# ThomasHelfer/multimodal-supernovae

Hardware: AMD Instinct MI355X
Metric: contrastive pairs/sec (image+light-curve) at global batch 1024, 1/2/4/8 GPUs (higher is better)
Workload: dtype f32; 1 GPU; ViT-S/8 image tower (64x64x3, build-defined) + reference light-curve transformer (T=200, emb 64, 8 heads, depth 5, 2 bands) -> enc_dim 128, symmetric InfoNCE with all-gathered global negatives, RAdam; full train step; per_gpu_batch=1024, global_batch=1024, parallelism=dp1, launch=eager, gemm_precision=bf16x6

## Files before the change

include/msn_hip.h:

```cpp
#ifndef MSN_HIP_H
#define MSN_HIP_H

#include <stddef.h>
#include <stdint.h>

#ifdef __cplusplus
extern "C" {
#endif

#define MSN_OK 0
#define MSN_ERR_SHAPE 1
#define MSN_ERR_HIP 2

typedef void* msn_stream_t;

int msn_version(void);
const char* msn_last_error(void);
int msn_clock_probe(unsigned long long* out2, int microseconds, msn_stream_t stream);
int msn_device_count(void);

#define MSN_OP_N 0
#define MSN_OP_T 1
#define MSN_EPI_NONE 0
#define MSN_EPI_RELU 1
// ... 86 lines not shown
                       msn_stream_t stream);
size_t msn_time_embed_bwd_workspace_bytes(int64_t B, int e, int nband);
int msn_time_embed_bwd(const float* dy, const float* x, int64_t B, int T, int e, int nband, float* dw,
                       float* dbw, float* dband, void* ws, size_t ws_bytes, msn_stream_t stream);

#define MSN_POOL_MEAN 0
#define MSN_POOL_MAX 1
int msn_masked_pool_fwd(const float* x, const uint8_t* mask, int64_t B, int T, int e, int mode, float* out,
                        int* argmax, float* count, msn_stream_t stream);
int msn_masked_pool_bwd(const float* dout, const uint8_t* mask, int64_t B, int T, int e, int mode,
                        const int* argmax, const float* count, float* dx, msn_stream_t stream);
int msn_mask_tokens(const float* x, const uint8_t* mask, int64_t rows, int e, float* y, msn_stream_t stream);

int msn_add_rows(float* dst, int64_t ldd, const float* src, int64_t lds, int64_t rows, int cols, msn_stream_t stream);

size_t msn_plane_bytes(int64_t R, int64_t C, int planes);
size_t msn_plane_split_colsum_workspace_bytes(int64_t R, int64_t C);
int msn_plane_split(const float* x, int64_t ldx, int64_t R, int64_t C, int planes, int transposed, void* out, float* colsum,
                    void* ws, size_t ws_bytes, msn_stream_t stream);
typedef struct msn_split_item {
    const float* x;
    int64_t ldx, R, C;
    int transposed;
    void* out;
} msn_split_item;
int msn_plane_split_list(int n, const msn_split_item* items, int planes, msn_stream_t stream);
int msn_plane_merge(const void* planes_in, int planes, int64_t R, int64_t C, float* y, int64_t ldy, msn_stream_t stream);
size_t msn_pgemm_nt_colsum_workspace_bytes(int64_t M, int N);
size_t msn_pgemm_nt_workspace_bytes(int64_t M, int N, int K, int planes, int c_planes, int epilogue, int want_colsum);
int msn_set_pgemm_tail_split(int enabled);
int msn_pgemm_nt(int64_t M, int N, int K, int planes, const void* A, const void* B, void* C, int64_t ldc, int c_planes,
                 const float* bias, int epilogue, float* aux, int64_t ldaux, float* colsum_out, void* ws, size_t ws_bytes,
                 msn_stream_t stream);
size_t msn_pgemm_tn_workspace_bytes(int64_t M, int N, int K, int planes);
int msn_pgemm_tn(int64_t M, int N, int K, int planes, const void* A, const void* B, float* C, int64_t ldc, void* ws,
                 size_t ws_bytes, msn_stream_t stream);
int msn_layernorm_fwd_planes(const float* x, int64_t ldx, int64_t rows, int cols, const float* gamma, const float* beta,
                             float eps, int planes, void* y_planes, float* y, int64_t ldy, float* mean, float* rstd,
                             msn_stream_t stream);
int msn_layernorm_bwd_planes(const float* dy, int64_t lddy, const float* x, int64_t ldx, int64_t rows, int cols,
                             const float* mean, const float* rstd, const float* gamma, const float* add, int64_t ldadd,
                             float* dx, int64_t lddx, int planes, void* dx_planes, float* dgamma, float* dbeta,
                             float* dx_colsum, void* ws, size_t ws_bytes, msn_stream_t stream);
int msn_attention_fwd_planes(const float* qkv, int64_t ldqkv, const uint8_t* key_mask, int B, int H, int T, int head_dim,
                             float scale, float* out, int64_t ldo, float* lse, int planes, void* out_planes, msn_stream_t stream);
size_t msn_attention_bwd_planes_workspace_bytes(int B, int H, int head_dim);
int msn_attention_bwd_planes(const float* qkv, int64_t ldqkv, const uint8_t* key_mask, int B, int H, int T, int head_dim,
                             float scale, const float* out, int64_t ldo, const float* lse, const float* dout, int64_t ldd,
                             int planes, void* dqkv_planes, float* colsum_out, void* ws, size_t ws_bytes,
                             msn_stream_t stream);
int msn_plane_split_f16(const float* x, int64_t ldx, int64_t R, int64_t C, int transposed, void* out, float* scale,
                        int reuse_scale, float* colsum, void* ws, size_t ws_bytes, msn_stream_t stream);
int msn_pgemm_nt_f16(int64_t M, int N, int K, const void* A, const float* scaleA, const void* B, const float* scaleB, float* C,
                     int64_t ldc, const float* bias, int epilogue, float* aux, int64_t ldaux, float* colsum_out, void* ws,
                     size_t ws_bytes, msn_stream_t stream);
int msn_pgemm_tn_f16(int64_t M, int N, int K, const void* A, const float* scaleA, const void* B, const float* scaleB, float* C,
                     int64_t ldc, void* ws, size_t ws_bytes, msn_stream_t stream);

int msn_ffn_supported(int64_t M, int emb, int hidden);
int msn_ffn_fwd(const float* x, int64_t ldx, int64_t M, int emb, int hidden, const void* w1_planes, const void* w2t_planes,
                const float* c1, const float* c2, float* z, int64_t ldz, msn_stream_t stream);
size_t msn_ffn_bwd_workspace_bytes(int64_t M, int emb, int hidden);
int msn_ffn_bwd(const float* x, int64_t ldx, const float* dz, int64_t lddz, int64_t M, int emb, int hidden, const void* w1_planes,
                const void* w2t_planes, const float* c1, float* dx, int64_t lddx, float* dw1, float* dc1, float* dw2, float* dc2,
                void* ws, size_t ws_bytes, msn_stream_t stream);

// ... 224 lines not shown
```

multimodal_supernovae_amd/_lib.py:

```python
import ctypes
import os

import torch

_HERE = os.path.dirname(os.path.abspath(__file__))
LIB_PATH = os.environ.get("MSN_HIP_LIB") or os.path.join(_HERE, "lib", "libmsn_hip.so")

c_i64 = ctypes.c_int64
c_int = ctypes.c_int
c_f32 = ctypes.c_float
c_f64 = ctypes.c_double
c_ptr = ctypes.c_void_p
c_size = ctypes.c_size_t

SIGNATURES = {
    "msn_version": (c_int, []),
    "msn_last_error": (ctypes.c_char_p, []),
    "msn_clock_probe": (c_int, [c_ptr, c_int, c_ptr]),
    "msn_ffn_supported": (c_int, [c_i64, c_int, c_int]),
    "msn_ffn_fwd": (c_int, [c_ptr, c_i64, c_i64, c_int, c_int, c_ptr, c_ptr, c_ptr, c_ptr, c_ptr, c_i64, c_ptr]),
    "msn_ffn_bwd_workspace_bytes": (c_size, [c_i64, c_int, c_int]),
    "msn_ffn_bwd": (c_int, [c_ptr, c_i64, c_ptr, c_i64, c_i64, c_int, c_int, c_ptr, c_ptr, c_ptr, c_ptr, c_i64, c_ptr, c_ptr, c_ptr,
                            c_ptr, c_ptr, c_size, c_ptr]),
    "msn_cls_attention_supported": (c_int, [c_int, c_int]),
# ... 25 lines not shown
    "msn_colsum_workspace_bytes": (c_size, [c_i64, c_i64]),
    "msn_colsum": (c_int, [c_ptr, c_i64, c_i64, c_i64, c_ptr, c_ptr, c_size, c_ptr]),
    "msn_layernorm_fwd": (c_int, [c_ptr, c_i64, c_i64, c_int, c_ptr, c_ptr, c_f32, c_ptr, c_i64, c_ptr, c_ptr, c_ptr]),
    "msn_layernorm_bwd_workspace_bytes": (c_size, [c_i64, c_int]),
    "msn_layernorm_bwd": (c_int, [c_ptr, c_i64, c_ptr, c_i64, c_i64, c_int, c_ptr, c_ptr, c_ptr, c_ptr, c_i64,
                                  c_ptr, c_i64, c_ptr, c_ptr, c_ptr, c_size, c_ptr]),
    "msn_vit_tokens_fwd": (c_int, [c_ptr, c_ptr, c_ptr, c_i64, c_int, c_int, c_ptr, c_ptr]),
    "msn_vit_tokens_bwd": (c_int, [c_ptr, c_i64, c_int, c_int, c_ptr, c_ptr]),
    "msn_l2norm_fwd": (c_int, [c_ptr, c_i64, c_i64, c_int, c_ptr, c_i64, c_ptr, c_ptr]),
    "msn_l2norm_bwd": (c_int, [c_ptr, c_i64, c_ptr, c_i64, c_i64, c_int, c_ptr, c_ptr, c_i64, c_ptr]),
    "msn_time_embed_fwd": (c_int, [c_ptr, c_ptr, c_i64, c_int, c_int, c_ptr, c_ptr, c_ptr, c_ptr, c_int, c_ptr,
                                   c_ptr]),
    "msn_time_embed_bwd_workspace_bytes": (c_size, [c_i64, c_int, c_int]),
    "msn_time_embed_bwd": (c_int, [c_ptr, c_ptr, c_i64, c_int, c_int, c_int, c_ptr, c_ptr, c_ptr, c_ptr, c_size,
                                   c_ptr]),
    "msn_masked_pool_fwd": (c_int, [c_ptr, c_ptr, c_i64, c_int, c_int, c_int, c_ptr, c_ptr, c_ptr, c_ptr]),
    "msn_masked_pool_bwd": (c_int, [c_ptr, c_ptr, c_i64, c_int, c_int, c_int, c_ptr, c_ptr, c_ptr, c_ptr]),
    "msn_mask_tokens": (c_int, [c_ptr, c_ptr, c_i64, c_int, c_ptr, c_ptr]),
    "msn_add_rows": (c_int, [c_ptr, c_i64, c_ptr, c_i64, c_i64, c_int, c_ptr]),
    "msn_plane_bytes": (c_size, [c_i64, c_i64, c_int]),
    "msn_plane_split_colsum_workspace_bytes": (c_size, [c_i64, c_i64]),
    "msn_plane_split": (c_int, [c_ptr, c_i64, c_i64, c_i64, c_int, c_int, c_ptr, c_ptr, c_ptr, c_size, c_ptr]),
    "msn_plane_split_list": (c_int, [c_int, c_ptr, c_int, c_ptr]),
    "msn_plane_split_f16": (c_int, [c_ptr, c_i64, c_i64, c_i64, c_int, c_ptr, c_ptr, c_int, c_ptr, c_ptr, c_size, c_ptr]),
    "msn_pgemm_nt_f16": (c_int, [c_i64, c_int, c_int, c_ptr, c_ptr, c_ptr, c_ptr, c_ptr, c_i64, c_ptr, c_int, c_ptr, c_i64, c_ptr,
                                 c_ptr, c_size, c_ptr]),
    "msn_pgemm_tn_f16": (c_int, [c_i64, c_int, c_int, c_ptr, c_ptr, c_ptr, c_ptr, c_ptr, c_i64, c_ptr, c_size, c_ptr]),
    "msn_plane_merge": (c_int, [c_ptr, c_int, c_i64, c_i64, c_ptr, c_i64, c_ptr]),
    "msn_pgemm_nt_colsum_workspace_bytes": (c_size, [c_i64, c_int]),
    "msn_pgemm_nt_workspace_bytes": (c_size, [c_i64, c_int, c_int, c_int, c_int, c_int, c_int]),
    "msn_set_pgemm_tail_split": (c_int, [c_int]),
    "msn_pgemm_nt": (c_int, [c_i64, c_int, c_int, c_int, c_ptr, c_ptr, c_ptr, c_i64, c_int, c_ptr, c_int, c_ptr, c_i64, c_ptr,
                             c_ptr, c_size, c_ptr]),
    "msn_pgemm_tn_workspace_bytes": (c_size, [c_i64, c_int, c_int, c_int]),
    "msn_pgemm_tn": (c_int, [c_i64, c_int, c_int, c_int, c_ptr, c_ptr, c_ptr, c_i64, c_ptr, c_size, c_ptr]),
    "msn_layernorm_fwd_planes": (c_int, [c_ptr, c_i64, c_i64, c_int, c_ptr, c_ptr, c_f32, c_int, c_ptr, c_ptr, c_i64, c_ptr, c_ptr,
                                         c_ptr]),
    "msn_layernorm_bwd_planes": (c_int, [c_ptr, c_i64, c_ptr, c_i64, c_i64, c_int, c_ptr, c_ptr, c_ptr, c_ptr, c_i64, c_ptr,
                                         c_i64, c_int, c_ptr, c_ptr, c_ptr, c_ptr, c_ptr, c_size, c_ptr]),
    "msn_bgemm_nt": (c_int, [c_i64, c_int, c_int, c_ptr, c_i64, c_ptr, c_i64, c_ptr, c_i64, c_int, c_ptr, c_int, c_ptr, c_i64,
                             c_ptr, c_ptr, c_size, c_ptr]),
    "msn_bgemm_nt_colsum_workspace_bytes": (c_size, [c_i64, c_int]),
    "msn_bgemm_tn_workspace_bytes": (c_size, [c_i64, c_int, c_int]),
    "msn_bgemm_tn": (c_int, [c_i64, c_int, c_int, c_ptr, c_i64, c_ptr, c_i64, c_ptr, c_i64, c_ptr, c_size, c_ptr]),
    "msn_cast_bf16": (c_int, [c_ptr, c_i64, c_ptr, c_ptr]),
    "msn_attention_bf16_fwd": (c_int, [c_ptr, c_i64, c_int, c_int, c_int, c_f32, c_ptr, c_i64, c_ptr, c_ptr]),
    "msn_attention_bf16_bwd": (c_int, [c_ptr, c_i64, c_ptr, c_i64, c_ptr, c_i64, c_ptr, c_int, c_int, c_int, c_f32, c_ptr,
                                       c_ptr, c_ptr, c_ptr, c_ptr]),
    "msn_cast_bf16_transposed": (c_int, [c_ptr, c_int, c_int, c_ptr, c_ptr]),
    "msn_bcolsum_workspace_bytes": (c_size, [c_i64, c_int]),
    "msn_bcolsum": (c_int, [c_ptr, c_i64, c_i64, c_int, c_ptr, c_ptr, c_size, c_ptr]),
    "msn_layernorm_fwd_bf16": (c_int, [c_ptr, c_i64, c_i64, c_int, c_ptr, c_ptr, c_f32, c_ptr, c_i64, c_ptr, c_ptr, c_ptr]),
    "msn_layernorm_bwd_bf16": (c_int, [c_ptr, c_i64, c_ptr, c_i64, c_i64, c_int, c_ptr, c_ptr, c_ptr, c_ptr, c_i64, c_ptr,
                                       c_i64, c_ptr, c_ptr, c_ptr, c_ptr, c_int, c_ptr, c_size, c_ptr]),
    "msn_attention_fwd": (c_int, [c_ptr, c_i64, c_i64, c_ptr, c_i64, c_i64, c_ptr, c_i64, c_i64, c_ptr,
                                  c_int, c_int, c_int, c_int, c_int, c_f32, c_ptr, c_i64, c_i64, c_ptr, c_ptr]),
    "msn_attention_bwd": (c_int, [c_ptr, c_i64, c_i64, c_ptr, c_i64, c_i64, c_ptr, c_i64, c_i64, c_ptr,
                                  c_int, c_int, c_int, c_int, c_int, c_f32, c_ptr, c_i64, c_i64, c_ptr,
                                  c_ptr, c_i64, c_i64, c_ptr, c_ptr, c_i64, c_i64, c_ptr, c_i64, c_i64,
                                  c_ptr, c_i64, c_i64, c_ptr]),
    "msn_patchify": (c_int, [c_ptr, c_int, c_int, c_int, c_int, c_int, c_ptr, c_ptr]),
    "msn_unpatchify": (c_int, [c_ptr, c_int, c_int, c_int, c_int, c_int, c_ptr, c_ptr]),
    "msn_bn_workspace_bytes": (c_size, [c_i64, c_int]),
    "msn_batchnorm_fwd": (c_int, [c_ptr, c_i64, c_int, c_ptr, c_ptr, c_f32, c_int, c_f32, c_ptr, c_ptr, c_ptr, c_int,
                                  c_ptr, c_ptr, c_ptr, c_ptr, c_size, c_ptr]),
    "msn_dropout": (c_int, [c_ptr, c_i64, c_f32, ctypes.c_uint64, c_ptr, c_ptr, c_ptr]),
# ... 145 lines not shown
```

multimodal_supernovae_amd/csrc/pgemm.hip:

```cpp


#include "pgemm_kernels.h"

namespace msn {
extern template __global__ void pgemm_nt_kernel<2, 128, true, false, 2, 4, false>(const PgemmArgs);
extern template __global__ void pgemm_nt_kernel<2, 128, false, false, 2, 4, false>(const PgemmArgs);
extern template __global__ void pgemm_nt_kernel<2, 128, false, true, 4, 2, false, true>(const PgemmArgs);
extern template __global__ void pgemm_tn_kernel<2, 128, true, false, 2, 4>(const PgemmArgs);
extern template __global__ void pgemm_tn_kernel<2, 128, false, false, 2, 4>(const PgemmArgs);
extern template __global__ void pgemm_tn_kernel<2, 128, true, true, 2, 4, true>(const PgemmArgs);
extern template __global__ void pgemm_tn_kernel<2, 128, false, true, 2, 4, true>(const PgemmArgs);
}

namespace msn {

__global__ __launch_bounds__(256) void pgemm_tail_finish_kernel(const PgemmArgs p, int bn) {
    const int tiles_tail = p.tiles_m * p.tiles_n - p.tail_full;
    const int per_tile = BM * bn / 4;
    const int64_t i = (int64_t)blockIdx.x * 256 + threadIdx.x;
    if (i >= (int64_t)tiles_tail * per_tile) return;
    const int tt = (int)(i / per_tile), e = (int)(i % per_tile);
    int tm, tn;
    nt_locate(p, p.tail_full + tt, tm, tn);
    const int row = e / (bn / 4), c4 = e % (bn / 4);
    const int64_t m = (int64_t)tm * BM + row;
    const int n = tn * bn + 4 * c4;
    if (m >= p.M || n >= p.N) return;
    float4 s = make_float4(0.f, 0.f, 0.f, 0.f);
    for (int g = 0; g < p.tail_segs; ++g) {
        const float4 v = *reinterpret_cast<const float4*>(p.tail_slabs + ((int64_t)(tt * p.tail_segs + g) * BM + row) * bn + 4 * c4);
        s.x += v.x; s.y += v.y; s.z += v.z; s.w += v.w;
    }
    if (p.bias) {
        const float4 b = *reinterpret_cast<const float4*>(p.bias + n);
        s.x += b.x; s.y += b.y; s.z += b.z; s.w += b.w;
    }
    if (p.epi == MSN_EPI_ADD) {
        const float4 a = *reinterpret_cast<const float4*>(p.aux + m * p.ldaux + n);
        s.x += a.x; s.y += a.y; s.z += a.z; s.w += a.w;
    } else if (p.epi == MSN_EPI_RELU) {
        s.x = fmaxf(s.x, 0.f); s.y = fmaxf(s.y, 0.f); s.z = fmaxf(s.z, 0.f); s.w = fmaxf(s.w, 0.f);
    }
    *reinterpret_cast<float4*>(static_cast<float*>(p.C) + m * p.ldc + n) = s;
}
// ... 500 lines not shown
    } else {
        launch_nt<2, 128, false>(a, c_planes != 0, grid, st);
    }
    MSN_LAUNCH_CHECK();
    if (a.tail_segs) {
        const int64_t threads = (int64_t)(total - a.tail_full) * (BM * bn / 4);
        hipLaunchKernelGGL(pgemm_tail_finish_kernel, dim3((unsigned)cdiv(threads, 256)), dim3(256), 0, st, a, bn);
        MSN_LAUNCH_CHECK();
    }
    if (colsum_after) return msn_colsum(static_cast<const float*>(C), ldc, M, N, colsum_out, ws, ws_bytes, stream);
    if (colsum_out) {
        if (colsum_finish(a.colpart, (a.colsum_rows ? a.colsum_rows : 2) * a.tiles_m, N, colsum_out, st) != MSN_OK) {
            set_error("msn_pgemm_nt: column-sum launch failed");
            return MSN_ERR_HIP;
        }
    }
    return MSN_OK;
}

extern "C" int msn_pgemm_nt(int64_t M, int N, int K, int planes, const void* A, const void* B, void* C, int64_t ldc,
                            int c_planes, const float* bias, int epilogue, float* aux, int64_t ldaux, float* colsum_out,
                            void* ws, size_t ws_bytes, msn_stream_t stream) {
    return pgemm_nt_impl(M, N, K, planes, A, B, C, ldc, c_planes, bias, epilogue, aux, ldaux, colsum_out, ws, ws_bytes, stream,
                         nullptr, nullptr);
}
extern "C" int msn_pgemm_nt_f16(int64_t M, int N, int K, const void* A, const float* scaleA, const void* B, const float* scaleB,
                                float* C, int64_t ldc, const float* bias, int epilogue, float* aux, int64_t ldaux,
                                float* colsum_out, void* ws, size_t ws_bytes, msn_stream_t stream) {
    MSN_REQUIRE(scaleA && scaleB, "msn_pgemm_nt_f16: the operands' scales are missing");
    return pgemm_nt_impl(M, N, K, 2, A, B, C, ldc, 0, bias, epilogue, aux, ldaux, colsum_out, ws, ws_bytes, stream, scaleA, scaleB);
}

namespace {
struct TnPlan { bool swap; int bq, tiles_p, tiles_q, splits, rb_per_split; };
TnPlan tn_plan(int64_t M, int N, int K, int planes) {
    TnPlan t;
    auto waste = [](int n, int w) { return (int)(cdiv(n, w) * w - n); };
    const int wn = waste(N, 256), wk = waste(K, 256);
    t.swap = wk < wn;
    const int Pd = t.swap ? K : N, Qd = t.swap ? N : K;
    t.bq = 128;
    t.tiles_p = (int)cdiv(Pd, 256);
    t.tiles_q = (int)cdiv(Qd, t.bq);
    const int tiles = t.tiles_p * t.tiles_q;
    const int rbs = (int)cdiv(M, 32);
    int s = std::max(1, 256 / tiles);
    const int64_t rb_bytes = 2 * std::max(cdiv(N, 32), cdiv(K, 32)) * (int64_t)planes * 1024;
    s = (int)std::max<int64_t>(s, cdiv(rbs, std::max<int64_t>(1, ((1ll << 31) - 1) / rb_bytes)));
    s = std::min(s, rbs);
    t.rb_per_split = (int)cdiv(rbs, s);
    t.splits = (int)cdiv(rbs, t.rb_per_split);
    return t;
}
}

extern "C" size_t msn_pgemm_tn_workspace_bytes(int64_t M, int N, int K, int planes) {
    if (M <= 0 || N <= 0 || K <= 0) return 0;
    const TnPlan t = tn_plan(M, N, K, planes);
    return t.splits > 1 ? sizeof(float) * (size_t)t.splits * N * K : 0;
}

template <int NP, int BQ, bool DUAL, int WM = 2, int WN = 4, int FOLDN = 1>
static void launch_tn(const PgemmArgs& a, bool swap, int grid, hipStream_t st) {
    if (swap) hipLaunchKernelGGL((pgemm_tn_kernel<NP, BQ, true, DUAL, WM, WN, false, FOLDN>), dim3((unsigned)grid), dim3(512), 0, st, a);
    else hipLaunchKernelGGL((pgemm_tn_kernel<NP, BQ, false, DUAL, WM, WN, false, FOLDN>), dim3((unsigned)grid), dim3(512), 0, st, a);
}

static int pgemm_tn_impl(int64_t M, int N, int K, int planes, const void* A, const void* B, float* C, int64_t ldc, void* ws,
                         size_t ws_bytes, msn_stream_t stream, const float* scaleA, const float* scaleB) {
    const bool f16 = scaleA != nullptr;
    MSN_REQUIRE(M > 0 && N > 0 && K > 0 && A && B && C, "msn_pgemm_tn: empty operand");
    MSN_REQUIRE(!f16 || (scaleB && planes == 2), "msn_pgemm_tn_f16: two fp16 planes per operand, both scales");
    MSN_REQUIRE(planes == 2 || planes == 3, "msn_pgemm_tn: planes must be 2 or 3 (got %d)", planes);
    MSN_REQUIRE(K % 4 == 0 && ldc >= K && ldc % 4 == 0 && aligned16(C, A, B),
                "msn_pgemm_tn: K and ldc must be multiples of 4, operands 16-byte aligned");
    MSN_REQUIRE(std::max(N, K) < (1 << 19), "msn_pgemm_tn: N and K must be below 2^19 (32-bit offsets inside a row block of planes)");
    const TnPlan t = tn_plan(M, N, K, planes);
    PgemmArgs a = {};
    a.A = static_cast<const unsigned char*>(A); a.B = static_cast<const unsigned char*>(B); a.C = C;
    a.ldc = ldc; a.M = M; a.N = N; a.K = K;
    a.rbA = a.rbB = (int)cdiv(M, 32);
    a.cbA = 2 * (int)cdiv(N, 32); a.cbB = 2 * (int)cdiv(K, 32);
    a.tiles_m = t.tiles_p; a.tiles_n = t.tiles_q;
    a.splits = t.splits; a.rb_per_split = t.rb_per_split;
    const size_t need = t.splits > 1 ? sizeof(float) * (size_t)t.splits * N * K : 0;
    MSN_REQUIRE(need == 0 || (ws && ws_bytes >= need && aligned16(ws)), "msn_pgemm_tn: workspace %zu < %zu bytes", ws_bytes, need);
    a.slabs = static_cast<float*>(ws);
    a.scaleA = scaleA, a.scaleB = scaleB;
    const int grid = t.tiles_p * t.tiles_q * t.splits;
    hipStream_t st = static_cast<hipStream_t>(stream);
    if (planes == 3) launch_tn<3, 128, true, 2, 4, 2>(a, t.swap, grid, st);
    else if (f16 && t.swap) hipLaunchKernelGGL((pgemm_tn_kernel<2, 128, true, true, 2, 4, true>), dim3((unsigned)grid), dim3(512), 0, st, a);
    else if (f16) hipLaunchKernelGGL((pgemm_tn_kernel<2, 128, false, true, 2, 4, true>), dim3((unsigned)grid), dim3(512), 0, st, a);
    else launch_tn<2, 128, false>(a, t.swap, grid, st);
    MSN_LAUNCH_CHECK();
    if (t.splits > 1) {
        const int64_t n4 = (int64_t)N * K / 4;
        if (int rc = slab_sum(a.slabs, t.splits, n4, K / 4, ldc / 4, C, st)) return rc;
    }
    return MSN_OK;
}

extern "C" int msn_pgemm_tn(int64_t M, int N, int K, int planes, const void* A, const void* B, float* C, int64_t ldc, void* ws,
                            size_t ws_bytes, msn_stream_t stream) {
    return pgemm_tn_impl(M, N, K, planes, A, B, C, ldc, ws, ws_bytes, stream, nullptr, nullptr);
}
extern "C" int msn_pgemm_tn_f16(int64_t M, int N, int K, const void* A, const float* scaleA, const void* B, const float* scaleB,
                                float* C, int64_t ldc, void* ws, size_t ws_bytes, msn_stream_t stream) {
    MSN_REQUIRE(scaleA && scaleB, "msn_pgemm_tn_f16: the operands' scales are missing");
    return pgemm_tn_impl(M, N, K, 2, A, B, C, ldc, ws, ws_bytes, stream, scaleA, scaleB);
}
```

multimodal_supernovae_amd/csrc/pgemm_alt2.hip:

```cpp
#include "pgemm_kernels.h"

namespace msn {
template __global__ void pgemm_nt_kernel<2, 128, true, false, 2, 4, false>(const PgemmArgs);
template __global__ void pgemm_nt_kernel<2, 128, false, false, 2, 4, false>(const PgemmArgs);
template __global__ void pgemm_nt_kernel<2, 128, false, true, 4, 2, false, true>(const PgemmArgs);
template __global__ void pgemm_tn_kernel<2, 128, true, false, 2, 4>(const PgemmArgs);
template __global__ void pgemm_tn_kernel<2, 128, false, false, 2, 4>(const PgemmArgs);
template __global__ void pgemm_tn_kernel<2, 128, true, true, 2, 4, true>(const PgemmArgs);
template __global__ void pgemm_tn_kernel<2, 128, false, true, 2, 4, true>(const PgemmArgs);
}
```

multimodal_supernovae_amd/csrc/pgemm_kernels.h:

```cpp
#pragma once
#include <algorithm>
#include <type_traits>
#include "msn_common.h"

namespace msn {

typedef _Float16 f16x8 __attribute__((ext_vector_type(8)));
typedef unsigned u32x4 __attribute__((ext_vector_type(4)));
typedef unsigned u32x2 __attribute__((ext_vector_type(2)));
typedef __attribute__((address_space(1))) const void gptr_t;
typedef __attribute__((address_space(3))) void lptr_t;

#ifndef MSN_PG_ST_AUX
#define MSN_PG_ST_AUX 0
#endif
constexpr int BM = 256;

struct PgemmArgs {
    const unsigned char* A;
    const unsigned char* B;
    void* C;
    float* aux;
    const float* bias;
    int64_t ldc, ldaux;
// ... 639 lines not shown
            for (int k = kb; k < ke; k += 2) {
                step(T0{});
                step(T1{}, k + 2 >= ke);
            }
            wait_lgkm<0>();
            store_tile_epi(tm, tn, std::integral_constant<int, MSN_EPI_NONE>{}, std::integral_constant<int, 2 + 8>{});
            req_first_settled((unsigned)(c_slot * SLOT));
            continue;
        }
        int k0 = 0;
        for (; k0 + csteps < nk; k0 += csteps) {
            for (int k = 0; k < csteps; k += 2) {
                step(T0{});
                step(T1{}, k + 2 >= csteps);
            }
            wait_lgkm<0>();
            if (k0 == 0) store_tile_epi(tm, tn, std::integral_constant<int, MSN_EPI_NONE>{}, std::integral_constant<int, 2>{});
            else store_tile_epi(tm, tn, std::integral_constant<int, MSN_EPI_NONE>{}, std::integral_constant<int, 3>{});
            zero_acc();
            req_first_settled((unsigned)(c_slot * SLOT));
        }
        for (int k = k0; k < nk; k += 2) {
            step(T0{});
            step(T1{}, k + 2 >= nk);
        }
        wait_lgkm<0>();
        if (k0 != 0) store_tile(tm, tn, std::integral_constant<int, 1>{});
        else if (p.colpart) store_tile(tm, tn, std::integral_constant<int, 4>{});
        else store_tile(tm, tn, std::integral_constant<int, 0>{});
        req_first_settled((unsigned)(c_slot * SLOT));
    }
}

template <int NP, int BQ, bool SWAP, bool DUAL, int WM = 2, int WN = 4, bool F16 = false, int FOLDN = 1>
__global__ __launch_bounds__(512, 2) void pgemm_tn_kernel(const PgemmArgs p) {
    static_assert(WM * WN == 8, "eight waves");
    constexpr int PHB = 16 * NP, QHB = (BQ / 16) * NP;
    constexpr int PIECES = (PHB + QHB) / 2;
    constexpr int PP = PHB / 2;
    constexpr int SLOT = PIECES * PBLK;
    constexpr int NSLOT = (4 * SLOT <= 160 * 1024) ? 4 : 3;
    constexpr int MAXQ = (PIECES + 7) / 8;
    constexpr int MT = 8 / WM, NT = BQ / (32 * WN);
    constexpr int NG = NP * (NP + 1) / 2;
    __shared__ __attribute__((aligned(1024))) unsigned char lds[NSLOT * SLOT];

    const int lane = threadIdx.x & 63;
    const int wave = __builtin_amdgcn_readfirstlane(threadIdx.x >> 6);
    const int wm = wave / WN, wn = wave % WN;
    const int tiles = p.tiles_m * p.tiles_n;
    int bid = blockIdx.x;
    {
        const int nwg = gridDim.x, q = nwg / 8, r = nwg % 8, x = bid % 8, i = bid / 8;
        bid = (x < r ? x * (q + 1) : r * (q + 1) + (x - r) * q) + i;
    }
    const int split = bid / tiles, tile = bid % tiles;
    const int tp = tile / p.tiles_n, tq = tile % p.tiles_n;
    const unsigned char* Pm = SWAP ? p.B : p.A;
    const unsigned char* Qm = SWAP ? p.A : p.B;
    const int cbP = SWAP ? p.cbB : p.cbA, cbQ = SWAP ? p.cbA : p.cbB;
    const int rb0 = split * p.rb_per_split;
    const int rb1 = min(p.rbA, rb0 + p.rb_per_split);
    const int nk = 2 * (rb1 - rb0);

    const int sub = lane >> 5, j = lane & 31;
    typedef __amdgpu_buffer_rsrc_t rsrc_t;
    auto uniform_rsrc = [&](const unsigned char* base, int64_t bytes) -> rsrc_t {
        const uint64_t a = reinterpret_cast<uint64_t>(base);
        const unsigned lo = __builtin_amdgcn_readfirstlane((unsigned)a), hi = __builtin_amdgcn_readfirstlane((unsigned)(a >> 32));
        const int nb = __builtin_amdgcn_readfirstlane((int)min<int64_t>(bytes, 0x7fffffff));
        return __builtin_amdgcn_make_buffer_rsrc(reinterpret_cast<void*>(((uint64_t)hi << 32) | lo), (short)0, nb, 0x00020000);
    };
    const int64_t rbstepP = (int64_t)cbP * (NP * PBLK), rbstepQ = (int64_t)cbQ * (NP * PBLK);
    const rsrc_t rsP = uniform_rsrc(Pm + ((int64_t)rb0 * cbP + tp * 16) * (NP * PBLK), (int64_t)(rb1 - rb0) * rbstepP);
    const rsrc_t rsQ = uniform_rsrc(Qm + ((int64_t)rb0 * cbQ + tq * (BQ / 16)) * (NP * PBLK), (int64_t)(rb1 - rb0) * rbstepQ);
    unsigned plane_off[MAXQ];
#pragma unroll
    for (int q = 0; q < MAXQ; ++q) {
        const int id = min(wave + 8 * q, PIECES - 1);
        const bool isP = id < PP;
        const int hb = 2 * (isP ? id : id - PP) + sub;
        const int cbp = hb / NP;
        const int cb0 = isP ? tp * 16 : tq * (BQ / 16);
        const int cbs = isP ? cbP : cbQ;
        const int hbc = min(hb, (cbs - cb0) * NP - 1);
        const int rpos = j >> 1;
        const int rsrc = (rpos & 3) + 4 * ((rpos >> 2) ^ (cbp & 1));
        plane_off[q] = (unsigned)(hbc * PBLK + rsrc * 32 + (j & 1) * 16);
    }
    int p_k = 0, p_slot = 0;
    auto issue_q = [&](int q) {
        const int id = wave + 8 * q;
        if (id < PIECES) {
            const int soff = (int)((p_k >> 1) * (id < PP ? rbstepP : rbstepQ)) + (p_k & 1) * 512;
            __builtin_amdgcn_raw_ptr_buffer_load_lds(id < PP ? rsP : rsQ, (lptr_t*)(lds + p_slot * SLOT + id * PBLK), 16, (int)plane_off[q], soff, 0, 0);
        }
    };
    auto issue_chunk = [&](auto c_) {
        constexpr int c = decltype(c_)::value;
        if (p_k < nk) {
#pragma unroll
            for (int q = c * MAXQ / NG; q < (c + 1) * MAXQ / NG; ++q) issue_q(q);
        }
    };
    auto advance = [&]() {
        if (p_k < nk) {
            ++p_k;
            p_slot = (p_slot + 1 == NSLOT) ? 0 : p_slot + 1;
        }
    };
    constexpr int Q_BEFORE = (NG - 1) * MAXQ / NG;
    const int ppw = (wave + 8 * (MAXQ - 1) < PIECES) ? MAXQ : MAXQ - 1;

    const int g16 = (lane >> 4) & 1, moct = lane >> 5, rq = (lane >> 2) & 3, pp = lane & 3;
    const unsigned lds0 = (unsigned)(uintptr_t)(lptr_t*)lds;
    const unsigned tr0 = lds0 + (unsigned)(g16 * NP * 512 + ((2 * moct) ^ g16) * 128 + rq * 32 + pp * 8);
    const unsigned tr1 = lds0 + (unsigned)(g16 * NP * 512 + ((2 * moct + 1) ^ g16) * 128 + rq * 32 + pp * 8);
    const unsigned fragP0 = tr0 + (unsigned)(wm * 2 * MT * NP * 512), fragP1 = tr1 + (unsigned)(wm * 2 * MT * NP * 512);
    const unsigned fragQ0 = tr0 + (unsigned)(PHB * 512 + wn * 2 * NT * NP * 512), fragQ1 = tr1 + (unsigned)(PHB * 512 + wn * 2 * NT * NP * 512);

    f32x16 acc[MT][NT], acc2[DUAL ? MT : 1][DUAL ? NT : 1];
#pragma unroll
    for (int i = 0; i < MT; ++i)
#pragma unroll
        for (int jj = 0; jj < NT; ++jj)
#pragma unroll
            for (int e = 0; e < 16; ++e) {
                acc[i][jj][e] = 0.f;
                if constexpr (DUAL) acc2[i][jj][e] = 0.f;
            }
    bf16x4 fa[2][MT][2], fb0[2][NT][2], fbh[NP > 1 ? NP - 1 : 1][NT][2];

    auto req_a = [&](bf16x4 (&dst)[MT][2], unsigned slot_off, auto pl_) {
        constexpr int pl = decltype(pl_)::value;
        static_for<0, MT>([&](auto i_) {
            constexpr int i = decltype(i_)::value;
            ds_read_tr_o<(2 * i * NP + pl) * 512>(dst[i][0], fragP0 + slot_off);
            ds_read_tr_o<(2 * i * NP + pl) * 512>(dst[i][1], fragP1 + slot_off);
        });
    };
    auto req_b = [&](bf16x4 (&dst)[NT][2], unsigned slot_off, auto pl_) {
        constexpr int pl = decltype(pl_)::value;
        static_for<0, NT>([&](auto j_) {
            constexpr int jj = decltype(j_)::value;
            ds_read_tr_o<(2 * jj * NP + pl) * 512>(dst[jj][0], fragQ0 + slot_off);
            ds_read_tr_o<(2 * jj * NP + pl) * 512>(dst[jj][1], fragQ1 + slot_off);
        });
    };
    auto mfma1 = [&](const bf16x8& av, const bf16x8& bv, const f32x16& c) -> f32x16 {
        if constexpr (F16) {
            const f16x8 ha = __builtin_bit_cast(f16x8, av), hb = __builtin_bit_cast(f16x8, bv);
            if constexpr (SWAP) return __builtin_amdgcn_mfma_f32_32x32x16_f16(ha, hb, c, 0, 0, 0);
// ... 102 lines not shown
                mult(fa[QA], fbh[pb - 1], SML{});
                if constexpr (DUAL && pb == 1) fold_pending();
            }
            issue_chunk(std::integral_constant<int, pb>{});
            __builtin_amdgcn_sched_barrier(0);
        });
        static_for<1, NP - 1>([&](auto pa_) {
            constexpr int pa = decltype(pa_)::value;
            constexpr int g0 = pa * NP - pa * (pa - 1) / 2;
            req_a(fa[(QA + pa + 1) & 1], cur, std::integral_constant<int, pa + 1>{});
            wait_lgkm<2 * MT>();
            static_for<0, NP - pa>([&](auto pb_) {
                constexpr int pb = decltype(pb_)::value;
                if constexpr (pb == 0) mult(fa[(QA + pa) & 1], fb0[PAR], SML{});
                else mult(fa[(QA + pa) & 1], fbh[pb - 1], SML{});
                issue_chunk(std::integral_constant<int, g0 + pb>{});
                __builtin_amdgcn_sched_barrier(0);
            });
        });
        wait_lgkm<0>();
        wait_vm(p_was_live ? (NSLOT - 3) * ppw + Q_BEFORE : 0);
        __builtin_amdgcn_s_barrier();
        __builtin_amdgcn_sched_barrier(0);
        req_a(fa[(QA + NP) & 1], nxt, std::integral_constant<int, 0>{});
        req_b(fb0[PAR ^ 1], nxt, std::integral_constant<int, 0>{});
        __builtin_amdgcn_sched_barrier(0);
        mult(fa[(QA + NP - 1) & 1], fb0[PAR], SML{});
        issue_chunk(std::integral_constant<int, NG - 1>{});
        __builtin_amdgcn_sched_barrier(0);
        advance();
        c_slot = n_slot;
    };

#pragma unroll
    for (int s_ = 0; s_ < NSLOT - 1; ++s_) {
        if (p_k < nk) {
#pragma unroll
            for (int q = 0; q < MAXQ; ++q) issue_q(q);
        }
        advance();
    }
    asm volatile("s_waitcnt vmcnt(0)" ::: "memory");
    __builtin_amdgcn_s_barrier();
    __builtin_amdgcn_sched_barrier(0);
    req_a(fa[0], 0u, std::integral_constant<int, 0>{});
    req_b(fb0[0], 0u, std::integral_constant<int, 0>{});
    for (int k = 0; k < nk; k += 2) {
        step(std::integral_constant<int, 0>{});
        step(std::integral_constant<int, 1>{});
    }
    wait_lgkm<0>();
    if constexpr (DUAL && FOLDN > 1) {
        fold(std::integral_constant<int, 1>{});
        fold(std::integral_constant<int, 3>{});
    }

    float* out = p.splits > 1 ? p.slabs + (int64_t)split * p.N * p.K : static_cast<float*>(p.C);
    const int64_t ldo = p.splits > 1 ? p.K : p.ldc;
    const int l31 = lane & 31, h4 = 4 * (lane >> 5);
    float os = 1.f;
    if constexpr (F16) os = p.scaleA[0] * p.scaleB[0];
#pragma unroll
    for (int i = 0; i < MT; ++i)
#pragma unroll
        for (int jj = 0; jj < NT; ++jj)
#pragma unroll
            for (int b = 0; b < 4; ++b) {
                int n, k;
                if constexpr (SWAP) {
                    k = tp * 256 + wm * (32 * MT) + 32 * i + 8 * b + h4;
                    n = tq * BQ + wn * (32 * NT) + 32 * jj + l31;
                } else {
                    n = tp * 256 + wm * (32 * MT) + 32 * i + l31;
                    k = tq * BQ + wn * (32 * NT) + 32 * jj + 8 * b + h4;
                }
                if (n >= p.N || k >= p.K) continue;
                float v[4];
#pragma unroll
                for (int r = 0; r < 4; ++r) {
                    v[r] = acc[i][jj][4 * b + r];
                    if constexpr (DUAL) v[r] += acc2[i][jj][4 * b + r];
                    if constexpr (F16) v[r] *= os;
                }
                *reinterpret_cast<float4*>(out + (int64_t)n * ldo + k) = make_float4(v[0], v[1], v[2], v[3]);
            }
}

}
```

multimodal_supernovae_amd/ops.py:

```python
import ctypes
import os

import torch

from . import _lib
from ._lib import check, lib, ptr, stream_ptr

GEMM_PROFILE = None
ATTN_PROFILE = None

PREC_F32, PREC_BF16X3, PREC_BF16 = 0, 1, 2
PREC_PLANES3, PREC_PLANES2 = 3, 4
_PREC_NAMES = {"f32": PREC_F32, "bf16x3": PREC_BF16X3, "bf16": PREC_BF16, "bf16x6": PREC_PLANES3, "bf16x3p": PREC_PLANES2}
_C_PRECISION = {PREC_F32: PREC_F32, PREC_BF16X3: PREC_BF16X3, PREC_BF16: PREC_BF16, PREC_PLANES3: PREC_F32,
                PREC_PLANES2: PREC_BF16X3}


def plane_count(precision=None):
    p = GEMM_PRECISION if precision is None else precision
    return 3 if p == PREC_PLANES3 else 2 if p == PREC_PLANES2 else 0
GEMM_PRECISION = _PREC_NAMES[os.environ.get("MSN_GEMM_PRECISION", "bf16x6").lower()]


class gemm_precision:
# ... 1152 lines not shown
    if want_colsum:
        out = out + (cs,)
    return out if len(out) > 1 else out[0]


def pgemm_tn(dy, x):
    assert isinstance(dy, Planes) and isinstance(x, Planes) and dy.R == x.R and dy.planes == x.planes
    M, N, K = dy.R, dy.C, x.C
    dev = dy.buf.device
    c = torch.empty((N, K), dtype=torch.float32, device=dev)
    L = lib()
    nb = L.msn_pgemm_tn_workspace_bytes(M, N, K, dy.planes)
    ws = _workspace(nb, dev) if nb else None
    nbytes = 2.0 * dy.planes * (M * N + M * K) + 4.0 * N * K
    with _span(GEMM_PROFILE, (2.0 * M * N * K, (OP_T, OP_N, N, K, M, 200), False, nbytes)):
        if dy.scale is not None:
            assert x.scale is not None
            check(L.msn_pgemm_tn_f16(M, N, K, ptr(dy.buf), ptr(dy.scale), ptr(x.buf), ptr(x.scale), ptr(c), K, ptr(ws), nb, stream_ptr()),
                  "msn_pgemm_tn_f16")
        else:
            check(L.msn_pgemm_tn(M, N, K, dy.planes, ptr(dy.buf), ptr(x.buf), ptr(c), K, ptr(ws), nb, stream_ptr()), "msn_pgemm_tn")
    return c


def layernorm_fwd_planes(x, gamma, beta, eps, planes):
    return _layernorm_fwd(x, gamma, beta, eps, planes=planes)


def layernorm_bwd_planes(dy, x, mean, rstd, gamma, planes, add=None, want_colsum=False):
    out = _layernorm_bwd(dy, x, mean, rstd, gamma, add, want_colsum, planes=planes)
    return out if want_colsum else out[:4]


def set_pgemm_tail_split(enabled):
    check(lib().msn_set_pgemm_tail_split(int(bool(enabled))))
```

Baseline: 15970 pairs/s.

## Pair split-K slices on ragged edge tiles in TN plane GEMM

Adds a paired variant of the weight-gradient (TN) plane GEMM for the 3-plane path. When the last P tile is at most half full, each of its two wave rows handles a different split-K slice, so one workgroup covers two splits. This lets the planner use more splits within 256 workgroups and cuts wasted work on the ragged edge tiles. The cost is a more complex tile-to-workgroup mapping, idle pipeline steps for the wave row with less work, and a larger LDS slot. Pairing is on by default and can be changed through an environment variable or a setter.

```diff
diff --git a/include/msn_hip.h b/include/msn_hip.h
--- a/include/msn_hip.h
+++ b/include/msn_hip.h
@@ -142,6 +142,8 @@
 int msn_pgemm_nt(int64_t M, int N, int K, int planes, const void* A, const void* B, void* C, int64_t ldc, int c_planes,
                  const float* bias, int epilogue, float* aux, int64_t ldaux, float* colsum_out, void* ws, size_t ws_bytes,
                  msn_stream_t stream);
+int msn_set_pgemm_tn_pairing(int mode);
+int msn_pgemm_tn_plan(int64_t M, int N, int K, int planes, int mode, int* info, int* wg, int wg_cap);
 size_t msn_pgemm_tn_workspace_bytes(int64_t M, int N, int K, int planes);
 int msn_pgemm_tn(int64_t M, int N, int K, int planes, const void* A, const void* B, float* C, int64_t ldc, void* ws,
                  size_t ws_bytes, msn_stream_t stream);
diff --git a/multimodal_supernovae_amd/_lib.py b/multimodal_supernovae_amd/_lib.py
--- a/multimodal_supernovae_amd/_lib.py
+++ b/multimodal_supernovae_amd/_lib.py
@@ -81,6 +81,8 @@
     "msn_set_pgemm_tail_split": (c_int, [c_int]),
     "msn_pgemm_nt": (c_int, [c_i64, c_int, c_int, c_int, c_ptr, c_ptr, c_ptr, c_i64, c_int, c_ptr, c_int, c_ptr, c_i64, c_ptr,
                              c_ptr, c_size, c_ptr]),
+    "msn_set_pgemm_tn_pairing": (c_int, [c_int]),
+    "msn_pgemm_tn_plan": (c_int, [c_i64, c_int, c_int, c_int, c_int, c_ptr, c_ptr, c_int]),
     "msn_pgemm_tn_workspace_bytes": (c_size, [c_i64, c_int, c_int, c_int]),
     "msn_pgemm_tn": (c_int, [c_i64, c_int, c_int, c_int, c_ptr, c_ptr, c_ptr, c_i64, c_ptr, c_size, c_ptr]),
     "msn_layernorm_fwd_planes": (c_int, [c_ptr, c_i64, c_i64, c_int, c_ptr, c_ptr, c_f32, c_int, c_ptr, c_ptr, c_i64, c_ptr, c_ptr,
diff --git a/multimodal_supernovae_amd/csrc/pgemm.hip b/multimodal_supernovae_amd/csrc/pgemm.hip
--- a/multimodal_supernovae_amd/csrc/pgemm.hip
+++ b/multimodal_supernovae_amd/csrc/pgemm.hip
@@ -1,5 +1,6 @@
 
 
+#include <cstdlib>
 #include "pgemm_kernels.h"
 
 namespace msn {
@@ -10,6 +11,8 @@
 extern template __global__ void pgemm_tn_kernel<2, 128, false, false, 2, 4>(const PgemmArgs);
 extern template __global__ void pgemm_tn_kernel<2, 128, true, true, 2, 4, true>(const PgemmArgs);
 extern template __global__ void pgemm_tn_kernel<2, 128, false, true, 2, 4, true>(const PgemmArgs);
+extern template __global__ void pgemm_tn_pair_kernel<3, 128, true, true, 2, 4, 2>(const PgemmArgs);
+extern template __global__ void pgemm_tn_pair_kernel<3, 128, false, true, 2, 4, 2>(const PgemmArgs);
 }
 
 namespace msn {
@@ -576,32 +579,74 @@
 }
 
 namespace {
-struct TnPlan { bool swap; int bq, tiles_p, tiles_q, splits, rb_per_split; };
-TnPlan tn_plan(int64_t M, int N, int K, int planes) {
+int g_tn_pairing = [] {
+    const char* e = std::getenv("MSN_PGEMM_TN_PAIRING");
+    return (e && e[0] >= '0' && e[0] <= '2' && !e[1]) ? e[0] - '0' : 1;
+}();
+
+#ifndef MSN_TN_PAIR_EDGE_DIV
+#define MSN_TN_PAIR_EDGE_DIV 3
+#endif
+struct TnPlan { bool swap, paired; int bq, tiles_p, tiles_q, splits, rb_per_split, grid; };
+TnPlan tn_plan(int64_t M, int N, int K, int planes, int mode) {
     TnPlan t;
     auto waste = [](int n, int w) { return (int)(cdiv(n, w) * w - n); };
     const int wn = waste(N, 256), wk = waste(K, 256);
     t.swap = wk < wn;
+    t.paired = false;
     const int Pd = t.swap ? K : N, Qd = t.swap ? N : K;
     t.bq = 128;
     t.tiles_p = (int)cdiv(Pd, 256);
     t.tiles_q = (int)cdiv(Qd, t.bq);
     const int tiles = t.tiles_p * t.tiles_q;
     const int rbs = (int)cdiv(M, 32);
-    int s = std::max(1, 256 / tiles);
     const int64_t rb_bytes = 2 * std::max(cdiv(N, 32), cdiv(K, 32)) * (int64_t)planes * 1024;
-    s = (int)std::max<int64_t>(s, cdiv(rbs, std::max<int64_t>(1, ((1ll << 31) - 1) / rb_bytes)));
-    s = std::min(s, rbs);
-    t.rb_per_split = (int)cdiv(rbs, s);
-    t.splits = (int)cdiv(rbs, t.rb_per_split);
+    const int64_t max_rb = ((1ll << 31) - 1) / rb_bytes;
+    auto split_into = [&](int s, int64_t span) {
+        s = (int)std::max<int64_t>(s, cdiv(rbs, std::max<int64_t>(1, span)));
+        s = std::min(s, rbs);
+        t.rb_per_split = (int)cdiv(rbs, s);
+        t.splits = (int)cdiv(rbs, t.rb_per_split);
+    };
+    split_into(std::max(1, 256 / tiles), max_rb);
+    t.grid = tiles * t.splits;
+    const int edge = t.tiles_q, full = tiles - edge;
+    if (mode != 0 && planes == 3 && Pd - 256 * (t.tiles_p - 1) <= 128 && MSN_TN_PAIR_EDGE_DIV * edge >= tiles && max_rb >= 2) {
+        const TnPlan t0 = t;
+        int s = 1;
+        while (full * (s + 1) + edge * ((s + 2) / 2) <= 256) ++s;
+        split_into(s, max_rb / 2);
+        t.grid = full * t.splits + edge * ((t.splits + 1) / 2);
+        if (t.splits < 2 || (t.grid > 256 && t0.grid <= 256)) return t0;
+        t.paired = mode == 1;
+        if (!t.paired) t.grid = tiles * t.splits;
+    }
     return t;
 }
+}
+
+extern "C" int msn_set_pgemm_tn_pairing(int mode) {
+    MSN_REQUIRE(mode >= 0 && mode <= 2, "msn_set_pgemm_tn_pairing: mode must be 0, 1 or 2 (got %d)", mode);
+    g_tn_pairing = mode;
+    return MSN_OK;
 }
 
 extern "C" size_t msn_pgemm_tn_workspace_bytes(int64_t M, int N, int K, int planes) {
     if (M <= 0 || N <= 0 || K <= 0) return 0;
-    const TnPlan t = tn_plan(M, N, K, planes);
+    const TnPlan t = tn_plan(M, N, K, planes, g_tn_pairing);
     return t.splits > 1 ? sizeof(float) * (size_t)t.splits * N * K : 0;
+}
+
+extern "C" int msn_pgemm_tn_plan(int64_t M, int N, int K, int planes, int mode, int* info, int* wg, int wg_cap) {
+    if (M <= 0 || N <= 0 || K <= 0 || (planes != 2 && planes != 3) || mode < 0 || mode > 2) return -1;
+    const TnPlan t = tn_plan(M, N, K, planes, mode);
+    if (info) {
+        const int v[8] = {t.swap, t.tiles_p, t.tiles_q, t.splits, t.rb_per_split, t.grid, t.paired, (int)cdiv(M, 32)};
+        std::copy(v, v + 8, info);
+    }
+    for (int i = 0; wg && i < std::min(t.grid, wg_cap); ++i)
+        tn_locate(t.paired, t.grid, i, t.tiles_p, t.tiles_q, t.splits, wg[4 * i], wg[4 * i + 1], wg[4 * i + 2], wg[4 * i + 3]);
+    return t.grid;
 }
 
 template <int NP, int BQ, bool DUAL, int WM = 2, int WN = 4, int FOLDN = 1>
@@ -619,7 +664,7 @@
     MSN_REQUIRE(K % 4 == 0 && ldc >= K && ldc % 4 == 0 && aligned16(C, A, B),
                 "msn_pgemm_tn: K and ldc must be multiples of 4, operands 16-byte aligned");
     MSN_REQUIRE(std::max(N, K) < (1 << 19), "msn_pgemm_tn: N and K must be below 2^19 (32-bit offsets inside a row block of planes)");
-    const TnPlan t = tn_plan(M, N, K, planes);
+    const TnPlan t = tn_plan(M, N, K, planes, g_tn_pairing);
     PgemmArgs a = {};
     a.A = static_cast<const unsigned char*>(A); a.B = static_cast<const unsigned char*>(B); a.C = C;
     a.ldc = ldc; a.M = M; a.N = N; a.K = K;
@@ -631,9 +676,11 @@
     MSN_REQUIRE(need == 0 || (ws && ws_bytes >= need && aligned16(ws)), "msn_pgemm_tn: workspace %zu < %zu bytes", ws_bytes, need);
     a.slabs = static_cast<float*>(ws);
     a.scaleA = scaleA, a.scaleB = scaleB;
-    const int grid = t.tiles_p * t.tiles_q * t.splits;
+    const int grid = t.grid;
     hipStream_t st = static_cast<hipStream_t>(stream);
-    if (planes == 3) launch_tn<3, 128, true, 2, 4, 2>(a, t.swap, grid, st);
+    if (t.paired && t.swap) hipLaunchKernelGGL((pgemm_tn_pair_kernel<3, 128, true, true, 2, 4, 2>), dim3((unsigned)grid), dim3(512), 0, st, a);
+    else if (t.paired) hipLaunchKernelGGL((pgemm_tn_pair_kernel<3, 128, false, true, 2, 4, 2>), dim3((unsigned)grid), dim3(512), 0, st, a);
+    else if (planes == 3) launch_tn<3, 128, true, 2, 4, 2>(a, t.swap, grid, st);
     else if (f16 && t.swap) hipLaunchKernelGGL((pgemm_tn_kernel<2, 128, true, true, 2, 4, true>), dim3((unsigned)grid), dim3(512), 0, st, a);
     else if (f16) hipLaunchKernelGGL((pgemm_tn_kernel<2, 128, false, true, 2, 4, true>), dim3((unsigned)grid), dim3(512), 0, st, a);
     else launch_tn<2, 128, false>(a, t.swap, grid, st);
diff --git a/multimodal_supernovae_amd/csrc/pgemm_alt2.hip b/multimodal_supernovae_amd/csrc/pgemm_alt2.hip
--- a/multimodal_supernovae_amd/csrc/pgemm_alt2.hip
+++ b/multimodal_supernovae_amd/csrc/pgemm_alt2.hip
@@ -8,4 +8,6 @@
 template __global__ void pgemm_tn_kernel<2, 128, false, false, 2, 4>(const PgemmArgs);
 template __global__ void pgemm_tn_kernel<2, 128, true, true, 2, 4, true>(const PgemmArgs);
 template __global__ void pgemm_tn_kernel<2, 128, false, true, 2, 4, true>(const PgemmArgs);
+template __global__ void pgemm_tn_pair_kernel<3, 128, true, true, 2, 4, 2>(const PgemmArgs);
+template __global__ void pgemm_tn_pair_kernel<3, 128, false, true, 2, 4, 2>(const PgemmArgs);
 }
diff --git a/multimodal_supernovae_amd/csrc/pgemm_kernels.h b/multimodal_supernovae_amd/csrc/pgemm_kernels.h
--- a/multimodal_supernovae_amd/csrc/pgemm_kernels.h
+++ b/multimodal_supernovae_amd/csrc/pgemm_kernels.h
@@ -695,36 +695,68 @@
     }
 }
 
-template <int NP, int BQ, bool SWAP, bool DUAL, int WM = 2, int WN = 4, bool F16 = false, int FOLDN = 1>
-__global__ __launch_bounds__(512, 2) void pgemm_tn_kernel(const PgemmArgs p) {
+template <int NP, int BQ, bool PAIR>
+struct TnShape {
+    static constexpr int PHB = 16 * NP, QHB = (BQ / 16) * NP;
+    static constexpr int PIECES = (PHB + (PAIR ? 2 : 1) * QHB) / 2;
+    static constexpr int SLOT = PIECES * PBLK;
+    static constexpr int NSLOT = (4 * SLOT <= 160 * 1024) ? 4 : 3;
+    static constexpr int LDS_BYTES = NSLOT * SLOT;
+};
+
+__host__ __device__ __forceinline__ void tn_locate(bool paired, int nwg, int wg, int tiles_p, int tiles_q, int splits, int& tp,
+                                                   int& tq, int& split, int& members) {
+    const int q = nwg / 8, r = nwg % 8, x = wg % 8, i = wg / 8;
+    const int bid = (x < r ? x * (q + 1) : r * (q + 1) + (x - r) * q) + i;
+    if (!paired) {
+        const int tiles = tiles_p * tiles_q, tile = bid % tiles;
+        split = bid / tiles;
+        tp = tile / tiles_q, tq = tile % tiles_q;
+        members = 1;
+        return;
+    }
+    const int F = (tiles_p - 1) * tiles_q, G = 2 * F + tiles_q;
+    const int jp = bid / G, u = bid % G;
+    const int two = 2 * jp + 1 < splits ? 2 : 1;
+    if (u < two * F) {
+        split = 2 * jp + u / F;
+        tp = (u % F) / tiles_q, tq = (u % F) % tiles_q;
+        members = 1;
+    } else {
+        split = 2 * jp;
+        tp = tiles_p - 1, tq = u - two * F;
+        members = two;
+    }
+}
+
+template <int NP, int BQ, bool SWAP, bool DUAL, int WM, int WN, bool F16, int FOLDN, bool PAIR>
+__device__ __forceinline__ void pgemm_tn_body(const PgemmArgs& p, unsigned char* lds, const int split, const int tp, const int tq,
+                                              const int members) {
     static_assert(WM * WN == 8, "eight waves");
-    constexpr int PHB = 16 * NP, QHB = (BQ / 16) * NP;
-    constexpr int PIECES = (PHB + QHB) / 2;
-    constexpr int PP = PHB / 2;
-    constexpr int SLOT = PIECES * PBLK;
-    constexpr int NSLOT = (4 * SLOT <= 160 * 1024) ? 4 : 3;
+    static_assert(!PAIR || WM == 2, "a pair is the two wave rows");
+    typedef TnShape<NP, BQ, PAIR> Shape;
+    constexpr int PHB = Shape::PHB, QHB = Shape::QHB;
+    constexpr int PIECES = Shape::PIECES;
+    constexpr int PP = PHB / 2, QP = QHB / 2;
+    constexpr int SLOT = Shape::SLOT;
+    constexpr int NSLOT = Shape::NSLOT;
     constexpr int MAXQ = (PIECES + 7) / 8;
     constexpr int MT = 8 / WM, NT = BQ / (32 * WN);
     constexpr int NG = NP * (NP + 1) / 2;
-    __shared__ __attribute__((aligned(1024))) unsigned char lds[NSLOT * SLOT];
 
     const int lane = threadIdx.x & 63;
     const int wave = __builtin_amdgcn_readfirstlane(threadIdx.x >> 6);
     const int wm = wave / WN, wn = wave % WN;
-    const int tiles = p.tiles_m * p.tiles_n;
-    int bid = blockIdx.x;
-    {
-        const int nwg = gridDim.x, q = nwg / 8, r = nwg % 8, x = bid % 8, i = bid / 8;
-        bid = (x < r ? x * (q + 1) : r * (q + 1) + (x - r) * q) + i;
-    }
-    const int split = bid / tiles, tile = bid % tiles;
-    const int tp = tile / p.tiles_n, tq = tile % p.tiles_n;
     const unsigned char* Pm = SWAP ? p.B : p.A;
     const unsigned char* Qm = SWAP ? p.A : p.B;
     const int cbP = SWAP ? p.cbB : p.cbA, cbQ = SWAP ? p.cbA : p.cbB;
     const int rb0 = split * p.rb_per_split;
     const int rb1 = min(p.rbA, rb0 + p.rb_per_split);
     const int nk = 2 * (rb1 - rb0);
+    const int rb2 = (PAIR && members == 2) ? min(p.rbA, rb1 + p.rb_per_split) : rb1;
+    const int nk1 = 2 * (rb2 - rb1);
+    const int my_nk = (PAIR && wm == 1) ? nk1 : nk;
+    const int k2_last = (nk1 > 0 ? nk1 : nk) - 1;
 
     const int sub = lane >> 5, j = lane & 31;
     typedef __amdgpu_buffer_rsrc_t rsrc_t;
@@ -735,8 +767,9 @@
         return __builtin_amdgcn_make_buffer_rsrc(reinterpret_cast<void*>(((uint64_t)hi << 32) | lo), (short)0, nb, 0x00020000);
     };
     const int64_t rbstepP = (int64_t)cbP * (NP * PBLK), rbstepQ = (int64_t)cbQ * (NP * PBLK);
-    const rsrc_t rsP = uniform_rsrc(Pm + ((int64_t)rb0 * cbP + tp * 16) * (NP * PBLK), (int64_t)(rb1 - rb0) * rbstepP);
-    const rsrc_t rsQ = uniform_rsrc(Qm + ((int64_t)rb0 * cbQ + tq * (BQ / 16)) * (NP * PBLK), (int64_t)(rb1 - rb0) * rbstepQ);
+    const rsrc_t rsP = uniform_rsrc(Pm + ((int64_t)rb0 * cbP + tp * 16) * (NP * PBLK), (int64_t)(rb2 - rb0) * rbstepP);
+    const rsrc_t rsQ = uniform_rsrc(Qm + ((int64_t)rb0 * cbQ + tq * (BQ / 16)) * (NP * PBLK), (int64_t)(rb2 - rb0) * rbstepQ);
+    auto second = [&](int id) { return PAIR && (id < PP ? id >= PP / 2 : id >= PP + QP); };
     unsigned plane_off[MAXQ];
 #pragma unroll
     for (int q = 0; q < MAXQ; ++q) {
@@ -744,18 +777,21 @@
         const bool isP = id < PP;
         const int hb = 2 * (isP ? id : id - PP) + sub;
         const int cbp = hb / NP;
+        const int hs = second(id) ? hb - (isP ? PHB / 2 : QHB) : hb;
         const int cb0 = isP ? tp * 16 : tq * (BQ / 16);
         const int cbs = isP ? cbP : cbQ;
-        const int hbc = min(hb, (cbs - cb0) * NP - 1);
+        const int hbc = min(hs, (cbs - cb0) * NP - 1);
         const int rpos = j >> 1;
         const int rsrc = (rpos & 3) + 4 * ((rpos >> 2) ^ (cbp & 1));
         plane_off[q] = (unsigned)(hbc * PBLK + rsrc * 32 + (j & 1) * 16);
+        if (second(id) && rb2 > rb1) plane_off[q] += (unsigned)((rb1 - rb0) * (isP ? rbstepP : rbstepQ));
     }
     int p_k = 0, p_slot = 0;
     auto issue_q = [&](int q) {
         const int id = wave + 8 * q;
         if (id < PIECES) {
-            const int soff = (int)((p_k >> 1) * (id < PP ? rbstepP : rbstepQ)) + (p_k & 1) * 512;
+            const int kk = second(id) ? min(p_k, k2_last) : p_k;
+            const int soff = (int)((kk >> 1) * (id < PP ? rbstepP : rbstepQ)) + (kk & 1) * 512;
             __builtin_amdgcn_raw_ptr_buffer_load_lds(id < PP ? rsP : rsQ, (lptr_t*)(lds + p_slot * SLOT + id * PBLK), 16, (int)plane_off[q], soff, 0, 0);
         }
     };
@@ -780,7 +816,8 @@
     const unsigned tr0 = lds0 + (unsigned)(g16 * NP * 512 + ((2 * moct) ^ g16) * 128 + rq * 32 + pp * 8);
     const unsigned tr1 = lds0 + (unsigned)(g16 * NP * 512 + ((2 * moct + 1) ^ g16) * 128 + rq * 32 + pp * 8);
     const unsigned fragP0 = tr0 + (unsigned)(wm * 2 * MT * NP * 512), fragP1 = tr1 + (unsigned)(wm * 2 * MT * NP * 512);
-    const unsigned fragQ0 = tr0 + (unsigned)(PHB * 512 + wn * 2 * NT * NP * 512), fragQ1 = tr1 + (unsigned)(PHB * 512 + wn * 2 * NT * NP * 512);
+    const unsigned q_reg = PAIR ? (unsigned)(wm * QHB * 512) : 0u;
+    const unsigned fragQ0 = tr0 + (unsigned)(PHB * 512 + wn * 2 * NT * NP * 512) + q_reg, fragQ1 = tr1 + (unsigned)(PHB * 512 + wn * 2 * NT * NP * 512) + q_reg;
 
     f32x16 acc[MT][NT], acc2[DUAL ? MT : 1][DUAL ? NT : 1];
 #pragma unroll
@@ -949,6 +986,20 @@
         c_slot = n_slot;
     };
 
+    auto idle_step = [&]() {
+        const bool p_was_live = p_k < nk;
+        wait_lgkm<0>();
+        static_for<0, NG - 1>([&](auto c_) { issue_chunk(c_); });
+        __builtin_amdgcn_sched_barrier(0);
+        wait_vm(p_was_live ? (NSLOT - 3) * ppw + Q_BEFORE : 0);
+        __builtin_amdgcn_s_barrier();
+        __builtin_amdgcn_sched_barrier(0);
+        issue_chunk(std::integral_constant<int, NG - 1>{});
+        __builtin_amdgcn_sched_barrier(0);
+        advance();
+        c_slot = (c_slot + 1 == NSLOT) ? 0 : c_slot + 1;
+    };
+
 #pragma unroll
     for (int s_ = 0; s_ < NSLOT - 1; ++s_) {
         if (p_k < nk) {
@@ -962,9 +1013,12 @@
     __builtin_amdgcn_sched_barrier(0);
     req_a(fa[0], 0u, std::integral_constant<int, 0>{});
     req_b(fb0[0], 0u, std::integral_constant<int, 0>{});
-    for (int k = 0; k < nk; k += 2) {
+    for (int k = 0; k < my_nk; k += 2) {
         step(std::integral_constant<int, 0>{});
         step(std::integral_constant<int, 1>{});
+    }
+    if constexpr (PAIR) {
+        for (int k = my_nk; k < nk; ++k) idle_step();
     }
     wait_lgkm<0>();
     if constexpr (DUAL && FOLDN > 1) {
@@ -972,9 +1026,11 @@
         fold(std::integral_constant<int, 3>{});
     }
 
-    float* out = p.splits > 1 ? p.slabs + (int64_t)split * p.N * p.K : static_cast<float*>(p.C);
+    if (PAIR && wm >= members) return;
+    float* out = p.splits > 1 ? p.slabs + (int64_t)(split + (PAIR ? wm : 0)) * p.N * p.K : static_cast<float*>(p.C);
     const int64_t ldo = p.splits > 1 ? p.K : p.ldc;
     const int l31 = lane & 31, h4 = 4 * (lane >> 5);
+    const int p0 = tp * 256 + (PAIR ? 0 : wm * (32 * MT));
     float os = 1.f;
     if constexpr (F16) os = p.scaleA[0] * p.scaleB[0];
 #pragma unroll
@@ -985,10 +1041,10 @@
             for (int b = 0; b < 4; ++b) {
                 int n, k;
                 if constexpr (SWAP) {
-                    k = tp * 256 + wm * (32 * MT) + 32 * i + 8 * b + h4;
+                    k = p0 + 32 * i + 8 * b + h4;
                     n = tq * BQ + wn * (32 * NT) + 32 * jj + l31;
                 } else {
-                    n = tp * 256 + wm * (32 * MT) + 32 * i + l31;
+                    n = p0 + 32 * i + l31;
                     k = tq * BQ + wn * (32 * NT) + 32 * jj + 8 * b + h4;
                 }
                 if (n >= p.N || k >= p.K) continue;
@@ -1003,4 +1059,22 @@
             }
 }
 
-}
+template <int NP, int BQ, bool SWAP, bool DUAL, int WM = 2, int WN = 4, bool F16 = false, int FOLDN = 1>
+__global__ __launch_bounds__(512, 2) void pgemm_tn_kernel(const PgemmArgs p) {
+    __shared__ __attribute__((aligned(1024))) unsigned char lds[TnShape<NP, BQ, false>::LDS_BYTES];
+    int tp, tq, split, members;
+    tn_locate(false, gridDim.x, blockIdx.x, p.tiles_m, p.tiles_n, p.splits, tp, tq, split, members);
+    pgemm_tn_body<NP, BQ, SWAP, DUAL, WM, WN, F16, FOLDN, false>(p, lds, split, tp, tq, 1);
+}
+
+template <int NP, int BQ, bool SWAP, bool DUAL, int WM = 2, int WN = 4, int FOLDN = 1>
+__global__ __launch_bounds__(512, 2) void pgemm_tn_pair_kernel(const PgemmArgs p) {
+    constexpr int LDS_BYTES = std::max(TnShape<NP, BQ, false>::LDS_BYTES, TnShape<NP, BQ, true>::LDS_BYTES);
+    __shared__ __attribute__((aligned(1024))) unsigned char lds[LDS_BYTES];
+    int tp, tq, split, members;
+    tn_locate(true, gridDim.x, blockIdx.x, p.tiles_m, p.tiles_n, p.splits, tp, tq, split, members);
+    if (tp + 1 < p.tiles_m) pgemm_tn_body<NP, BQ, SWAP, DUAL, WM, WN, false, FOLDN, false>(p, lds, split, tp, tq, 1);
+    else pgemm_tn_body<NP, BQ, SWAP, DUAL, WM, WN, false, FOLDN, true>(p, lds, split, tp, tq, members);
+}
+
+}
diff --git a/multimodal_supernovae_amd/ops.py b/multimodal_supernovae_amd/ops.py
--- a/multimodal_supernovae_amd/ops.py
+++ b/multimodal_supernovae_amd/ops.py
@@ -1208,5 +1208,20 @@
     return out if want_colsum else out[:4]
 
 
+def set_pgemm_tn_pairing(mode):
+    check(lib().msn_set_pgemm_tn_pairing(int(mode)), "msn_set_pgemm_tn_pairing")
+
+
+def pgemm_tn_plan(M, N, K, planes=3, mode=1):
+    import ctypes
+    info = (ctypes.c_int * 8)()
+    grid = lib().msn_pgemm_tn_plan(M, N, K, planes, mode, info, None, 0)
+    assert grid > 0, "msn_pgemm_tn_plan: bad arguments"
+    wg = (ctypes.c_int * (4 * grid))()
+    lib().msn_pgemm_tn_plan(M, N, K, planes, mode, info, wg, grid)
+    keys = ("swap", "tiles_p", "tiles_q", "splits", "rb_per_split", "grid", "paired", "row_blocks")
+    return dict(zip(keys, info)), [tuple(wg[4 * i:4 * i + 4]) for i in range(grid)]
+
+
 def set_pgemm_tail_split(enabled):
     check(lib().msn_set_pgemm_tail_split(int(bool(enabled))))
```

Result: no change. 16030 pairs/s, median of 6 (+0.3%).
